# MingSun-Tse/Collaborative-Distillation

Measured on AMD Instinct MI355X. Metric: content megapixels/sec, end-to-end 5-level WCT (16x VGG, 4K content, 2K style), higher is better.
Workload: dtype f32 (f16x3 split-MFMA products, fp32 accumulate); 1 GPU; PytorchWCT/WCT.py --mode 16x, 5-level WCT, 3840x2160 content, 2048x2048 style, alpha=1, style-side work included, images resident in HBM; BASELINE configs[1]; content_total=3840x2160, parallelism=content column strips x1

## Files before the change

collaborative-distillation_amd/csrc/solve.hip:

```cpp
#include "wct_common.h"
#include <cstdlib>

namespace {

typedef double f64x2 __attribute__((ext_vector_type(2)));
typedef unsigned u32x2 __attribute__((ext_vector_type(2)));

constexpr int MAX_SWEEPS = 40;
constexpr double ROT_TOL = 1e-12;
constexpr double ABS_FLOOR = 1e-13;
static const double REL_THRESH = [] { const char* e = wct_debug_env("WCT_REL_THRESH"); return e ? atof(e) : 1e-12; }();

__device__ __forceinline__ void tournament_pair(int n, int round, int k, int& p, int& q) {
  const int m = n - 1;
  if (k == 0) { p = m; q = round % m; }
  else { p = (round + k) % m; q = (round - k + m) % m; }
  if (p > q) { const int t = p; p = q; q = t; }
}

__device__ __forceinline__ double rsqrt_nr(double x) {
  double y = __builtin_amdgcn_rsq(x);
  y = y * (1.5 - 0.5 * x * y * y);
  y = y * (1.5 - 0.5 * x * y * y);
  return y;
// ... 336 lines not shown
    rows[((size_t)o * 9 + t) * cin + c] = v;
    ws += v;
  }
  wsum[e] = ws;
}

constexpr int COOP_NW = 32, COOP_MAXIT = 32;
struct NsSched { double ca[COOP_MAXIT], cb[COOP_MAXIT]; };
struct CoopArgs {
  int C; double n; const double* sum; const double* sumsq; double* res; double diag_add, eps_rel;
  NsWs w; int maxit, inverse; double zmax; int* info; int xcd;
  unsigned* coop_next;
  unsigned* aborts;
};
constexpr int BUF_SC1 = 16;
__device__ __forceinline__ unsigned xcc_id() { unsigned v; asm volatile("s_getreg_b32 %0, hwreg(HW_REG_XCC_ID)" : "=s"(v)); return v & 0xf; }
__device__ __forceinline__ __amdgpu_buffer_rsrc_t coop_rsrc(const void* p) {
  return __builtin_amdgcn_make_buffer_rsrc(const_cast<void*>(p), 0, 128 * 128 * 8, 0x00020000);
}
__device__ __forceinline__ f64x2 coop_ld2(__amdgpu_buffer_rsrc_t r, int elem) {
  return __builtin_bit_cast(f64x2, __builtin_amdgcn_raw_buffer_load_b128(r, elem * 8, 0, BUF_SC1));
}
__device__ __forceinline__ double coop_ld1(__amdgpu_buffer_rsrc_t r, int elem) {
  return __builtin_bit_cast(double, __builtin_amdgcn_raw_buffer_load_b64(r, elem * 8, 0, BUF_SC1));
}
__device__ __forceinline__ void coop_st1(__amdgpu_buffer_rsrc_t r, int elem, double v) {
  __builtin_amdgcn_raw_buffer_store_b64(__builtin_bit_cast(u32x2, v), r, elem * 8, 0, BUF_SC1);
}
__device__ __forceinline__ void gemm32_coop(const double* P, const double* Q, int i0, int j0, int lane, int wave, double (*red)[16 * 64], Acc32& acc) {
  constexpr int CP = 128;
  const int li = lane & 15, kk = lane >> 4, kbeg = wave * (CP / 4);
  const __amdgpu_buffer_rsrc_t rp = coop_rsrc(P), rq = coop_rsrc(Q);
#pragma unroll
  for (int t = 0; t < 4; ++t) acc.t[t] = f64x4{0., 0., 0., 0.};
  const int p0 = (i0 + li) * CP + 4 * kk, p1 = p0 + 16 * CP, q0 = (4 * kk) * CP + j0 + li;
  KBlock x[2];
#pragma unroll
  for (int b = 0; b < 2; ++b) {
    const int k0 = kbeg + 16 * b;
    x[b].a0l = coop_ld2(rp, p0 + k0); x[b].a0h = coop_ld2(rp, p0 + k0 + 2);
    x[b].a1l = coop_ld2(rp, p1 + k0); x[b].a1h = coop_ld2(rp, p1 + k0 + 2);
#pragma unroll
    for (int u = 0; u < 4; ++u) { x[b].b0[u] = coop_ld1(rq, q0 + (k0 + u) * CP); x[b].b1[u] = coop_ld1(rq, q0 + (k0 + u) * CP + 16); }
  }
  kblock_mfma(x[0], acc);
  kblock_mfma(x[1], acc);
  if (wave) {
#pragma unroll
    for (int t = 0; t < 4; ++t)
#pragma unroll
      for (int r = 0; r < 4; ++r) red[wave - 1][(t * 4 + r) * 64 + lane] = acc.t[t][r];
  }
  __syncthreads();
  if (!wave) {
#pragma unroll
    for (int t = 0; t < 4; ++t)
#pragma unroll
      for (int r = 0; r < 4; ++r) {
        const int at = (t * 4 + r) * 64 + lane;
        acc.t[t][r] = ((acc.t[t][r] + red[0][at]) + red[1][at]) + red[2][at];
      }
  }
  __syncthreads();
}
constexpr long long COOP_TIMEOUT_TICKS = 500000ll;
__device__ __forceinline__ void coop_abort(const NsWs& w, unsigned bit, unsigned* aborts) {
  const unsigned old = __hip_atomic_fetch_or(&w.coop[1], bit, __ATOMIC_RELAXED, __HIP_MEMORY_SCOPE_AGENT);
  if (old == 0u && aborts) __hip_atomic_fetch_add(aborts, 1u, __ATOMIC_RELAXED, __HIP_MEMORY_SCOPE_AGENT);
}
__device__ __forceinline__ bool coop_barrier(const NsWs& w, unsigned& target, int* ok_s, unsigned* aborts) {
  __builtin_amdgcn_s_waitcnt(0);
  __syncthreads();
  target += COOP_NW;
  if (threadIdx.x == 0) {
    __hip_atomic_fetch_add(&w.coop[0], 1u, __ATOMIC_RELAXED, __HIP_MEMORY_SCOPE_AGENT);
    const long long t0 = wall_clock64();
    bool ok = true;
    while (__hip_atomic_load(&w.coop[0], __ATOMIC_RELAXED, __HIP_MEMORY_SCOPE_AGENT) < target) {
      if (wall_clock64() - t0 > COOP_TIMEOUT_TICKS || __hip_atomic_load(&w.coop[1], __ATOMIC_RELAXED, __HIP_MEMORY_SCOPE_AGENT)) {
        coop_abort(w, 1u, aborts);
        ok = false;
        break;
      }
      __builtin_amdgcn_s_sleep(1);
    }
    *ok_s = ok;
  }
  __syncthreads();
  return *ok_s != 0;
}

__global__ __launch_bounds__(256) void ns_coop128_kernel(CoopArgs a, NsSched sc) {
  const bool inject = (a.xcd & 16) != 0;
  if ((int)(blockIdx.x & 7) != (a.xcd & 7)) return;
  constexpr int CP = 128;
  __shared__ double red[3][16 * 64];
  __shared__ int sdead[CP];
  __shared__ int ok_s;
  const NsWs& w = a.w;
  const int C = a.C, tid = threadIdx.x, me = blockIdx.x >> 3;
  const int lane = tid & 63, wave = tid >> 6, li = lane & 15, kk = lane >> 4;
  const double n = a.n;
  if (me == 0) {
    if (tid < 4) a.coop_next[tid] = 0u;
// ... 51 lines not shown
    const __amdgpu_buffer_rsrc_t ry = coop_rsrc(w.Y[0]), rz = coop_rsrc(w.Z[0]);
    for (int e = tid; e < 4 * CP; e += 256) {
      const int r = 4 * me + e / CP, c = e % CP;
      double y = r == c ? 1.0 : 0.0;
      if (r < C && c < C) {
        const double cv = cov_value(r, c, C, n, a.sum, a.sumsq, a.diag_add);
        a.res[(size_t)r * C + c] = cv;
        if (c == 0) a.res[(size_t)C * C + C + r] = a.sum[r] / n;
        if (!sdead[r] && !sdead[c]) y = (cv + (r == c ? s1 : 0.0)) / s0;
      }
      coop_st1(ry, r * CP + c, y);
      coop_st1(rz, r * CP + c, r == c ? 1.0 : 0.0);
    }
  }
  unsigned target = 0;
  if (!coop_barrier(w, target, &ok_s, a.aborts)) return;
  if (tid == 0 && (__hip_atomic_load(&w.coop[2], __ATOMIC_RELAXED, __HIP_MEMORY_SCOPE_AGENT) != xcc_id() + 1u || (inject && me == 7)))
    coop_abort(w, 2u, a.aborts);
  if (!coop_barrier(w, target, &ok_s, a.aborts)) return;
  if (__hip_atomic_load(&w.coop[1], __ATOMIC_RELAXED, __HIP_MEMORY_SCOPE_AGENT)) return;
  const int tile = me & 15, zside = me >> 4;
  const int i0 = (tile >> 2) * 32, j0 = (tile & 3) * 32;
  int nit = 0;
  for (int it = 0; it < a.maxit; ++it) {
    if (it > 0 && __longlong_as_double((long long)__hip_atomic_load(&w.resid[it - 1], __ATOMIC_RELAXED, __HIP_MEMORY_SCOPE_AGENT)) < NS_TOL) break;
    const int cur = it & 1, nxt = cur ^ 1;
    if (!zside) {
      Acc32 acc;
      gemm32_coop(w.Z[cur], w.Y[cur], i0, j0, lane, wave, red, acc);
      if (!wave) {
        const __amdgpu_buffer_rsrc_t rt = coop_rsrc(w.T);
        const double ca = sc.ca[it], cb = sc.cb[it];
        double m = 0.;
#pragma unroll
        for (int t = 0; t < 4; ++t)
#pragma unroll
          for (int r = 0; r < 4; ++r) {
            const int row = i0 + 16 * (t >> 1) + kk + 4 * r, col = j0 + 16 * (t & 1) + li;
            const double zy = acc.t[t][r], d = zy - (row == col ? 1.0 : 0.0);
            m = (d == d) ? fmax(m, fabs(d)) : __longlong_as_double(0x7ff0000000000000ll);
            coop_st1(rt, row * CP + col, (row == col ? ca : 0.0) - cb * zy);
          }
        for (int o = 32; o > 0; o >>= 1) m = fmax(m, __shfl_xor(m, o));
        if (lane == 0) atomicMax(&w.resid[it], (unsigned long long)__double_as_longlong(m));
      }
    }
    if (!coop_barrier(w, target, &ok_s, a.aborts)) return;
    {
      Acc32 acc;
      gemm32_coop(zside ? w.T : w.Y[cur], zside ? w.Z[cur] : w.T, i0, j0, lane, wave, red, acc);
      if (!wave) {
        const __amdgpu_buffer_rsrc_t ro = coop_rsrc(zside ? w.Z[nxt] : w.Y[nxt]);
#pragma unroll
        for (int t = 0; t < 4; ++t)
#pragma unroll
          for (int r = 0; r < 4; ++r) coop_st1(ro, (i0 + 16 * (t >> 1) + kk + 4 * r) * CP + j0 + 16 * (t & 1) + li, acc.t[t][r]);
        if (zside) {
          double q = 0.;
#pragma unroll
          for (int t = 0; t < 4; ++t) q += acc.t[t][0] * acc.t[t][0] + acc.t[t][1] * acc.t[t][1] + acc.t[t][2] * acc.t[t][2] + acc.t[t][3] * acc.t[t][3];
          for (int o = 32; o > 0; o >>= 1) q += __shfl_xor(q, o);
          if (lane == 0) atomicAdd(&w.zfro[it + 1], q);
        }
      }
    }
    if (!coop_barrier(w, target, &ok_s, a.aborts)) return;
    nit = it + 1;
  }
  bool ok = nit >= 1 && __longlong_as_double((long long)__hip_atomic_load(&w.resid[nit - 1], __ATOMIC_RELAXED, __HIP_MEMORY_SCOPE_AGENT)) < NS_TOL;
  if (ok && a.inverse) {
    const unsigned long long zb = __hip_atomic_load(reinterpret_cast<unsigned long long*>(&w.zfro[nit]), __ATOMIC_RELAXED, __HIP_MEMORY_SCOPE_AGENT);
    ok = __longlong_as_double((long long)zb) <= a.zmax * a.zmax;
  }
  if (me == 0 && tid == 0) { *w.iters = nit; *w.ok = ok ? 1 : 0; if (a.info && ok) *a.info = nit; }
  if (!ok) return;
  {
    const __amdgpu_buffer_rsrc_t rf = coop_rsrc(a.inverse ? w.Z[nit & 1] : w.Y[nit & 1]);
    const double sc_out = a.inverse ? rsqrt(s0) : sqrt(s0);
    for (int e = tid; e < 4 * CP; e += 256) {
      const int r = 4 * me + e / CP, c = e % CP;
      if (r >= C || c >= C) continue;
      double v = 0.;
      if (!sdead[r] && !sdead[c]) v = coop_ld1(rf, r * CP + c) * sc_out;
// ... 64 lines not shown
  const int li = lane & 15, kk = lane >> 4;
  f64x4 acc = f64x4{0., 0., 0., 0.};
  const double* pp = P + (i0 + li) * LD + kk;
  const double* qq = Q + kk * LD + j0 + li;
#pragma unroll 2
  for (int k0 = 0; k0 < CP; k0 += 16) {
    double a[4], b[4];
#pragma unroll
    for (int u = 0; u < 4; ++u) { a[u] = pp[k0 + 4 * u]; b[u] = qq[(k0 + 4 * u) * LD]; }
#pragma unroll
    for (int u = 0; u < 4; ++u) acc = __builtin_amdgcn_mfma_f64_16x16x4f64(a[u], b[u], acc, 0, 0, 0);
  }
  return acc;
}

template <int CP>
__global__ __launch_bounds__((CP / 16) * (CP / 16) * 64) void ns_lds_kernel(double* res, int C, int inverse, double eps_rel,
                                                                               int maxit, double zmax, int* ok_out, int* info,
                                                                               double npix, const double* sum, const double* sumsq, double diag_add,
                                                                               NsSched sched, int nsched) {
  constexpr int LD = CP + 2, TPR = CP / 16, NW = TPR * TPR, NT = NW * 64;
  extern __shared__ __attribute__((aligned(16))) char smem_ns[];
  double* Y = reinterpret_cast<double*>(smem_ns);
  double* Z = Y + CP * LD;
  double* T = Z + CP * LD;
  double* red = T + CP * LD;
  int* dead = reinterpret_cast<int*>(red + NW + 2);
  const int tid = threadIdx.x, lane = tid & 63, wave = __builtin_amdgcn_readfirstlane(tid >> 6);
  const int li = lane & 15, kk = lane >> 4;
  const int i0 = (wave / TPR) * 16, j0 = (wave % TPR) * 16;
  cov_by_block(C, npix, sum, sumsq, res, diag_add, tid, NT);
// ... 15 lines not shown
  if (!(f > 0.)) f = 1.;
  const double s = f * (1.0 + eps_rel), shift = eps_rel * f;
  for (int e = tid; e < CP * CP; e += NT) {
    const int r = e / CP, c = e - r * CP;
    double y = r == c ? 1.0 : 0.0;
    if (!dead[r] && !dead[c]) y = (res[(size_t)r * C + c] + (r == c ? shift : 0.0)) / s;
    Y[r * LD + c] = y;
    Z[r * LD + c] = r == c ? 1.0 : 0.0;
  }
  __syncthreads();
  int n = 0;
  double prev = 1e300;
  for (int it = 0; it < maxit; ++it) {
    if (it > 0 && prev < NS_TOL) break;
    const double ca = it < nsched ? sched.ca[it] : 1.5, cb = it < nsched ? sched.cb[it] : 0.5;
    const f64x4 zy = tile_gemm_lds<CP>(Z, Y, i0, j0, lane);
    double m = 0.;
#pragma unroll
    for (int r = 0; r < 4; ++r) {
      const int row = i0 + kk + 4 * r, col = j0 + li;
      const double d = zy[r] - (row == col ? 1.0 : 0.0);
      m = (d == d) ? fmax(m, fabs(d)) : __longlong_as_double(0x7ff0000000000000ll);
      T[row * LD + col] = (row == col ? ca : 0.0) - cb * zy[r];
    }
    for (int o = 32; o > 0; o >>= 1) m = fmax(m, __shfl_xor(m, o));
    if (lane == 0) red[wave] = m;
    __syncthreads();
    m = 0.;
    for (int w = 0; w < NW; ++w) m = fmax(m, red[w]);
    prev = m;
    const f64x4 yn = tile_gemm_lds<CP>(Y, T, i0, j0, lane);
    const f64x4 zn = tile_gemm_lds<CP>(T, Z, i0, j0, lane);
    __syncthreads();
#pragma unroll
    for (int r = 0; r < 4; ++r) {
      Y[(i0 + kk + 4 * r) * LD + j0 + li] = yn[r];
      Z[(i0 + kk + 4 * r) * LD + j0 + li] = zn[r];
    }
    __syncthreads();
    n = it + 1;
  }
  bool ok = n >= 1 && prev < NS_TOL;
  if (ok && inverse) {
    double q = 0.;
    for (int e = tid; e < CP * CP; e += NT) { const double z = Z[(e / CP) * LD + (e % CP)]; q += z * z; }
    for (int o = 32; o > 0; o >>= 1) q += __shfl_xor(q, o);
    __syncthreads();
    if (lane == 0) red[wave] = q;
    __syncthreads();
    q = 0.;
    for (int w = 0; w < NW; ++w) q += red[w];
    ok = q <= zmax * zmax;
// ... 224 lines not shown
  for (int j = threadIdx.x; j < n; j += 256) {
    const double l = lam[j];
    wj[j] = (l > thr && l > 0.) ? pow(l, expo - 2.0) : 0.;
  }
  __syncthreads();
  const long e = (long)blockIdx.x * blockDim.x + threadIdx.x;
  if (e >= (long)n * n) return;
  const int a = (int)(e / n), b = (int)(e % n);
  double s = 0.;
  for (int j = 0; j < n; ++j) s += wj[j] * G[(size_t)j * n + a] * G[(size_t)j * n + b];
  out[e] = s;
}

}

size_t eig_result_bytes(int C) { return eig_doubles(C) * sizeof(double); }
size_t eig_result_F_offset(size_t C) { return eig_F_offset((int)C); }
static inline int ns_pad(int C) { return C > 128 ? (C + 63) / 64 * 64 : (C + 31) / 32 * 32; }
size_t eig_workspace_bytes(int C) {
  const size_t cp2 = (size_t)ns_pad(C) * ns_pad(C);
  return 5 * cp2 * sizeof(double) + (size_t)C * sizeof(int) + 4 * sizeof(double) + 2 * (NS_MAXIT_REG + 2) * sizeof(unsigned long long) + 64;
}
size_t assemble_workspace_bytes(int C) { return (size_t)C * C * sizeof(double); }

bool eig_is_big(int C, bool wide_model) { return C > 128 || (wide_model && C > 64 && ns_pad(C) % 64 == 0); }

bool fold_gemm_capable(int cout, int cin, int cout_pad) { return cin >= 256 && cin % 128 == 0 && cout % 32 == 0 && cout_pad == cout; }
size_t fold_gemm_rows_doubles(int cout, int cin) { return (size_t)cout * 10 * cin; }

hipError_t launch_fold_rows(const float* w_oihw, int cout, int cin, double* rows, hipStream_t s) {
// ... 6 lines not shown
                            float* wpk_out, float* bias_out, unsigned* maxbits_dev, hipStream_t s) {
  if (!fold_gemm_capable(cout, cin, cout_pad)) return hipErrorInvalidValue;
  if (maxbits_dev) {
    hipError_t e = hipMemsetAsync(maxbits_dev, 0, sizeof(unsigned), s);
    if (e != hipSuccess) return e;
  }
  constexpr int NS = 8;
  const dim3 grid((unsigned)(cin / 32), (unsigned)(cout * 9 / 32 + (cout_pad + NS - 1) / NS));
  hipLaunchKernelGGL(fold_gemm_kernel<NS>, grid, dim3(64 * NS), 0, s, rows, rows + (size_t)cout * 9 * cin, bias, cout, cin, cout_pad, M, b, wpk_out,
                     bias_out, maxbits_dev);
  return hipGetLastError();
}

hipError_t launch_eig(int C, double n, const double* sum, const double* sumsq, int inverse, double* res, int* info_dev,
                      void* ws, size_t ws_bytes, hipStream_t s, double diag_add, bool wide_model, int* ok_defer, int coop_xcd, unsigned* coop_state, int* coop_epoch,
                      unsigned* coop_aborts, bool* coop_used_out, int sched_maxit, double sched_guess) {
  if (C < 2 || (C & 1) || C > 512 || n < 2) return hipErrorInvalidValue;
  if (ws_bytes < eig_workspace_bytes(C)) return hipErrorOutOfMemory;
  const size_t cc = (size_t)C * C;
  const int Cp = ns_pad(C);
  const size_t cp2 = (size_t)Cp * Cp;
  NsWs w;
  double* p = reinterpret_cast<double*>(ws);
  w.Y[0] = p; w.Y[1] = p + cp2; w.Z[0] = p + 2 * cp2; w.Z[1] = p + 3 * cp2; w.T = p + 4 * cp2;
  w.scal = p + 5 * cp2;
  w.resid = reinterpret_cast<unsigned long long*>(w.scal + 4);
  w.zfro = reinterpret_cast<double*>(w.resid + NS_MAXIT_REG + 2);
  w.iters = reinterpret_cast<int*>(w.zfro + NS_MAXIT_REG + 2);
  w.ok = w.iters + 1;
  w.coop = nullptr;
  w.dead = w.iters + 2;
// ... 15 lines not shown
      hipError_t e = hipFuncSetAttribute(reinterpret_cast<const void*>(kern), hipFuncAttributeMaxDynamicSharedMemorySize, (int)lds);
      if (e != hipSuccess) return e;
      NsSched sc;
      int nsched = 0;
      if (guess64 > 0.) {
        double xl = sqrt(guess64);
        for (; nsched < COOP_MAXIT && nsched < maxit; ++nsched) {
          const double mu = xl <= 0.9 ? sqrt(3.0 / (1.0 + xl + xl * xl)) : 1.0;
          xl = mu * xl * (3.0 - mu * mu * xl * xl) / 2.0;
          sc.ca[nsched] = 1.5 * mu; sc.cb[nsched] = 0.5 * mu * mu * mu;
        }
      }
      hipLaunchKernelGGL(kern, dim3(1), dim3((unsigned)nw * 64), lds, s, res, C, inverse, 1e-15, maxit, NS_ZMAX, w.ok, info_dev, n, sum, sumsq, diag_add, sc, nsched);
      return hipSuccess;
    };
    hipError_t e = Cp == 32 ? go(ns_lds_kernel<32>, 32) : go(ns_lds_kernel<64>, 64);
    if (e != hipSuccess) return e;
  } else {
    static const bool sk_env = [] { const char* e = wct_debug_env("WCT_NS_SPLITK"); return e ? atoi(e) != 0 : true; }();
    const bool splitk128 = sk_env && Cp % 64 == 0;
    const bool coop = !big && Cp == 128 && splitk128 && coop_xcd >= 0 && coop_state && coop_epoch && maxit <= COOP_MAXIT;
    coop_used = coop;
    if (coop_used_out) *coop_used_out = coop;
    if (coop) { w.coop = coop_state + 4 * (*coop_epoch & 1); ++*coop_epoch; }
    if (big) {
      hipLaunchKernelGGL(ns_init_kernel, dim3(1), dim3(1024), 0, s, res, C, NS_DEFLATE, w, maxit);
      hipLaunchKernelGGL(ns_fill_kernel, dim3((unsigned)((cp2 + 255) / 256)), dim3(256), 0, s, res, C, Cp, w);
    } else if (!coop) {
      hipLaunchKernelGGL(ns_prep_kernel, dim3(1), dim3(1024), 0, s, C, Cp, n, sum, sumsq, res, diag_add, 1e-15, w, maxit);
    }
    const dim3 g1(Cp / 32, Cp / 32, 1), g2(Cp / 32, Cp / 32, 2);
// ... 153 lines not shown
```

collaborative-distillation_amd/csrc/wct_api.hip:

```cpp
#include "../../include/wct_hip.h"
#include "../../include/wct_hip_color.h"
#include "../../include/wct_hip_smooth.h"
#include "../../include/wct_hip_swap.h"
#include "../../include/wct_hip_transform.h"
#include "wct_common.h"

#include <cmath>
#include <cstdarg>
#include <cstdlib>
#include <cstdio>
#include <atomic>
#include <cstring>
#include <dlfcn.h>
#include <map>
#include <mutex>
#include <string>
#include <vector>

namespace {

struct DevBuf {
  void* p = nullptr;
  size_t cap = 0;
};
// ... 46 lines not shown
  unsigned coop_solves = 0;
  bool coop_off = false;
};

struct wct_ctx {
  int device = 0;
  Lane main, side;
  hipEvent_t ev_join = nullptr;
  hipEvent_t ev_smom[6] = {nullptr, nullptr, nullptr, nullptr, nullptr, nullptr};
  hipEvent_t ev_sar[6] = {nullptr, nullptr, nullptr, nullptr, nullptr, nullptr};
  hipEvent_t ev_switch = nullptr;
  hipEvent_t ev_fork = nullptr, ev_style[6] = {nullptr, nullptr, nullptr, nullptr, nullptr, nullptr};
  int eig_skip = 0, eig_calls = 0;
  int foldgemm = 1;
  int nscoop = 1;
  int interleave = 1;
  std::string err;
  Module mod[2][6];
  DevBuf featC, featS, tmpT, wsAsm, small, foldW, foldW16, eigC, eigS[6];
  DevBuf foldS[6];
  bool fold_ready[6] = {false, false, false, false, false, false};
  int cur_level = 0, cur_h = 0, cur_w = 0;
  DevBuf u8c, u8s, u8o;
  DevBuf rsz_tmp;
  std::vector<ResizeAxis> rsz_axes;
  unsigned long long rsz_clock = 0;
  DevBuf noise;
  DevBuf colStyle, colOut, colWs;
  DevBuf smSums, smAB;
  DevBuf swFc, swFs, swQ, swK, swOut, swIdx, swRun, swNorm, swLab;
// ... 610 lines not shown
constexpr double OT_GUESS = 1e-10;

int eig_impl(wct_ctx* ctx, Lane& ln, int C, double n, const double* sum, const double* sumsq, int inverse, DevBuf& res, int* info_dev, bool ot_sched = false) {
  if (C < 2 || (C & 1) || C > 512) return fail(ctx, WCT_ERR_INVALID, "solve: C=%d must be even and <= 512", C);
  if (n < 2) return fail(ctx, WCT_ERR_INVALID, "solve: unbiased covariance needs >= 2 pixels (n=%g)", n);
  if (int rc = ensure(ctx, res, eig_result_bytes(C))) return rc;
  if (int rc = ensure(ctx, ln.wsEig, eig_workspace_bytes(C))) return rc;
  if (ctx->eig_skip > 0 && ++ctx->eig_calls > ctx->eig_skip) return WCT_OK;
  ProfScope ps(ctx, ln.stream, inverse ? "matfun_invsqrt" : "matfun_sqrt", 0, 0);
  int* defer = nullptr;
  if (ctx->defer_big && eig_is_big(C, ctx->wide_model) && ctx->ok_n < OK_SLOTS) defer = ctx->ok_log + ctx->ok_n++;
  const bool coop_ok = ctx->nscoop && coop_usable(ctx, ln);
  bool coop_used = false;
  HIPCHK(ctx, launch_eig(C, n, sum, sumsq, inverse, reinterpret_cast<double*>(res.p), info_dev, ln.wsEig.p, ln.wsEig.cap, ln.stream,
                         (inverse && ctx->numpy_variant && !ot_sched) ? 1.0 : 0.0, ctx->wide_model, defer, coop_ok ? (ln.xcd | (ctx->nscoop == 2 ? 16 : 0)) : -1, ln.coop, &ln.coop_epoch,
                         ctx->sat_dev + 2 + (&ln == &ctx->side ? 1 : 0), &coop_used, ot_sched ? OT_MAXIT : 0, ot_sched ? OT_GUESS : -1.0));
  if (coop_used) ++ln.coop_solves;
  return WCT_OK;
}

template <typename BODY>
int with_deferred_solves(wct_ctx* ctx, bool wait_side, BODY&& body) {
  if (!ctx->wide_model) return body();
  ctx->defer_big = true;
  ctx->ok_n = 0;
  HIPCHK(ctx, hipMemcpyAsync(ctx->sat_dev + 1, ctx->sat_dev, sizeof(unsigned), hipMemcpyDeviceToDevice, ctx->main.stream));
  int rc = body();
  ctx->defer_big = false;
  const int n = ctx->ok_n;
  ctx->ok_n = 0;
  if (rc) return rc;
// ... 392 lines not shown

int wct_debug_set(wct_ctx* ctx, const char* key, double value) {
  if (!ctx || !key) return WCT_ERR_INVALID;
  WCT_GUARD(ctx);
  const int v = value != 0.0;
  if (!strcmp(key, "fuse")) ctx->fuse = v;
  else if (!strcmp(key, "sp")) ctx->sp = v;
  else if (!strcmp(key, "l1fuse")) ctx->l1fuse = v;
  else if (!strcmp(key, "u8fuse")) ctx->u8fuse = v;
  else if (!strcmp(key, "upconv")) ctx->upconv = v;
  else if (!strcmp(key, "fastfold")) ctx->fastfold = v;
  else if (!strcmp(key, "interleave")) ctx->interleave = v;
  else if (!strcmp(key, "foldgemm")) ctx->foldgemm = v;
  else if (!strcmp(key, "prof_forms")) ctx->prof_forms = v;
  else if (!strcmp(key, "nscoop")) ctx->nscoop = (int)value;
  else if (!strcmp(key, "mom32")) ctx->mom32 = (int)value;
  else if (!strcmp(key, "in3wide")) ctx->in3wide = (int)value;
  else if (!strcmp(key, "poison")) {
    if (value < 0) { ctx->poison = -1; return WCT_OK; }
    if (value > 255 || value != (double)(int)value) return fail(ctx, WCT_ERR_INVALID, "debug_set: 'poison' takes a byte 0..255, or -1 for off");
    ctx->poison = (int)value;
    return poison_scratch(ctx, ctx->poison);
  }
  else if (!strcmp(key, "eig_skip")) {
    if (!getenv("WCT_DEBUG")) return fail(ctx, WCT_ERR_INVALID, "debug_set: 'eig_skip' produces wrong results by design (timing experiment); set WCT_DEBUG to allow it");
    ctx->eig_skip = (int)value; ctx->eig_calls = 0;
  }
  else if (!strcmp(key, "swap_key_chunk")) {
    if (!getenv("WCT_DEBUG")) return fail(ctx, WCT_ERR_INVALID, "debug_set: 'swap_key_chunk' is a test / measurement key; set WCT_DEBUG to allow it");
    if (value < 0 || value > 2147483647.0 || value != (double)(long)value) return fail(ctx, WCT_ERR_INVALID, "debug_set: 'swap_key_chunk' takes a key count >= 1, or 0 for the default");
// ... 7 lines not shown
    if (!ctx->coll_set || (ctx->comm_ranks != 1 && !ctx->shard_emulate)) return fail(ctx, WCT_ERR_STATE, "debug_set: 'shard_emulate' needs a ONE-rank communicator on the context");
    if (world < 2 || rank >= world) return fail(ctx, WCT_ERR_INVALID, "debug_set: 'shard_emulate' = 100 * ranks + rank");
    ctx->shard_emulate = true; ctx->comm_ranks = world; ctx->comm_rank = rank;
    return WCT_OK;
  }
  else if (!strcmp(key, "side_priority")) {
    int lo = 0, hi = 0;
    HIPCHK(ctx, hipDeviceGetStreamPriorityRange(&lo, &hi));
    HIPCHK(ctx, hipStreamSynchronize(ctx->side.stream));
    hipStream_t ns = nullptr;
    HIPCHK(ctx, hipStreamCreateWithPriority(&ns, hipStreamNonBlocking, value > 0 ? lo : (value < 0 ? hi : 0)));
    (void)hipStreamDestroy(ctx->side.stream);
    ctx->side.stream = ns;
    return WCT_OK;
  }
  else return fail(ctx, WCT_ERR_INVALID, "debug_set: unknown key '%s' (fuse, sp, l1fuse, u8fuse, upconv, fastfold, interleave, foldgemm, nscoop, in3wide, mom32, eig_skip, side_priority, poison, prof_forms, swap_key_chunk)", key);
  HIPCHK(ctx, hipStreamSynchronize(ctx->side.stream));
  return WCT_OK;
}

int wct_debug_get(wct_ctx* ctx, const char* key, double* value) {
  if (!ctx || !key || !value) return WCT_ERR_INVALID;
  WCT_GUARD(ctx);
  if (!strcmp(key, "nscoop_aborts") || !strcmp(key, "nscoop_solves") || !strcmp(key, "nscoop_off")) {
    if (!strcmp(key, "nscoop_solves")) { *value = (double)ctx->main.coop_solves + (double)ctx->side.coop_solves; return WCT_OK; }
    if (!strcmp(key, "nscoop_off")) { (void)coop_usable(ctx, ctx->main); (void)coop_usable(ctx, ctx->side); *value = (ctx->main.coop_off ? 1 : 0) + (ctx->side.coop_off ? 2 : 0); return WCT_OK; }
    HIPCHK(ctx, hipStreamSynchronize(ctx->side.stream));
    HIPCHK(ctx, hipStreamSynchronize(ctx->main.stream));
    unsigned n[2] = {0u, 0u};
    HIPCHK(ctx, hipMemcpy(n, ctx->sat_dev + 2, sizeof n, hipMemcpyDeviceToHost));
    if (ctx->sat_host) { reinterpret_cast<volatile unsigned*>(ctx->sat_host)[2] = n[0]; reinterpret_cast<volatile unsigned*>(ctx->sat_host)[3] = n[1]; }
// ... 1800 lines not shown
```

collaborative-distillation_amd/csrc/wct_common.h:

```cpp
#pragma once
#include <hip/hip_runtime.h>
#include <stdint.h>
#include <stddef.h>

#include <stdlib.h>
#include <vector>

typedef float f32x4 __attribute__((ext_vector_type(4)));
typedef double f64x4 __attribute__((ext_vector_type(4)));

static inline const char* wct_debug_env(const char* name) {
  const char* g = getenv("WCT_DEBUG");
  if (!g || !g[0] || (g[0] == '0' && !g[1])) return nullptr;
  return getenv(name);
}

struct LaunchForm { char form; int tile_h; bool multi; };
extern __thread LaunchForm wct_launch_form __attribute__((visibility("hidden")));
static inline void note_launch_form(char form, int tile_h, long units, long grid) {
  wct_launch_form.form = form; wct_launch_form.tile_h = tile_h; wct_launch_form.multi = units > grid;
}

__device__ __forceinline__ void sat_raise(unsigned* counter) {
  const unsigned old = atomicAdd(counter, 1u);
// ... 104 lines not shown
hipError_t launch_nhwc_to_nchw(const float* in, float* out, int C, int npix, hipStream_t s);
hipError_t launch_nchw_to_nhwc(const float* in, float* out, int C, int npix, hipStream_t s);

size_t moments_workspace_bytes(int C, long npix);
hipError_t launch_moments(const float* feat_nhwc, int C, int h, int wfull, int x0, int x1, double* sum,
                          double* sumsq, void* workspace, size_t workspace_bytes, hipStream_t s, bool f32_products = false);

size_t eig_result_bytes(int C);
size_t eig_result_F_offset(size_t C);
size_t eig_workspace_bytes(int C);
size_t assemble_workspace_bytes(int C);
bool eig_is_big(int C, bool wide_model);
hipError_t launch_eig(int C, double n, const double* sum, const double* sumsq, int inverse, double* res, int* info_dev,
                      void* workspace, size_t workspace_bytes, hipStream_t s, double diag_add = 0.0, bool wide_model = false,
                      int* ok_defer = nullptr, int coop_xcd = -1, unsigned* coop_state = nullptr, int* coop_epoch = nullptr, unsigned* coop_aborts = nullptr, bool* coop_used_out = nullptr,
                      int sched_maxit = 0, double sched_guess = -1.0);
hipError_t launch_assemble(int C, const double* eig_c, const double* eig_s, double alpha, double rel_thresh,
                           double* M, double* b, void* workspace, size_t workspace_bytes, hipStream_t s);

size_t ot_workspace_bytes(int C);
hipError_t launch_ot_sandwich(int C, double n, const double* sum_c, const double* sumsq_c, const double* S, double* B, double* zeros, double* tmp, hipStream_t s);
hipError_t launch_ot_assemble(int C, double alpha, const double* S, const double* mu_s, const double* Z, double n, const double* sum_c, double* tmp,
                              double* M, double* b, hipStream_t s);
hipError_t launch_adain_assemble(int C, double alpha, double eps, const double* S, const double* mu_s, double n, const double* sum_c, const double* sumsq_c,
                                 double* M, double* b, int* info_dev, hipStream_t s);

bool fold_gemm_capable(int cout, int cin, int cout_pad);
size_t fold_gemm_rows_doubles(int cout, int cin);
hipError_t launch_fold_rows(const float* w_oihw, int cout, int cin, double* rows, hipStream_t s);
hipError_t launch_fold_gemm(const double* rows, const float* bias, int cout, int cin, int cout_pad, const double* M, const double* b,
                            float* wpk_out, float* bias_out, unsigned* maxbits_dev, hipStream_t s);
// ... 34 lines not shown
```

Before: 1158 MP/s.

## Overlap Newton-Schulz operand loads with grid barriers and split LDS solver work

The cooperative Newton-Schulz kernel's grid barrier is split into arrive and wait, so operand loads for the second GEMM that do not depend on T are issued before the wait. The barrier poll reads the counter and abort flag together in one 64-bit load, one redundant barrier is removed, and the residual is cached per iteration. The single-block LDS solver gains a new form, on by default, that splits waves between the Y and Z updates and prefetches operands before the sync. Both kernels now use a DPP-based wave max reduction. Optional timing instrumentation is added under a compile flag.

Measured after the change: 1144 MP/s. -1.2%, worse.

```diff
diff --git a/collaborative-distillation_amd/csrc/solve.hip b/collaborative-distillation_amd/csrc/solve.hip
--- a/collaborative-distillation_amd/csrc/solve.hip
+++ b/collaborative-distillation_amd/csrc/solve.hip
@@ -5,6 +5,23 @@
 
 typedef double f64x2 __attribute__((ext_vector_type(2)));
 typedef unsigned u32x2 __attribute__((ext_vector_type(2)));
+
+template <int CTRL>
+__device__ __forceinline__ double dpp_f64(double v) {
+  const int lo = __builtin_amdgcn_update_dpp(0, __double2loint(v), CTRL, 0xf, 0xf, false);
+  const int hi = __builtin_amdgcn_update_dpp(0, __double2hiint(v), CTRL, 0xf, 0xf, false);
+  return __hiloint2double(hi, lo);
+}
+__device__ __forceinline__ double wave_fmax(double m) {
+  m = fmax(m, dpp_f64<0xB1>(m));
+  m = fmax(m, dpp_f64<0x4E>(m));
+  m = fmax(m, dpp_f64<0x141>(m));
+  m = fmax(m, dpp_f64<0x140>(m));
+  double r[4];
+#pragma unroll
+  for (int q = 0; q < 4; ++q) r[q] = __hiloint2double(__builtin_amdgcn_readlane(__double2hiint(m), 16 * q), __builtin_amdgcn_readlane(__double2loint(m), 16 * q));
+  return fmax(fmax(r[0], r[1]), fmax(r[2], r[3]));
+}
 
 constexpr int MAX_SWEEPS = 40;
 constexpr double ROT_TOL = 1e-12;
@@ -374,6 +391,26 @@
   unsigned* aborts;
 };
 constexpr int BUF_SC1 = 16;
+enum { NS_T_LOAD1, NS_T_MMA1, NS_T_RED1, NS_T_STORE1, NS_T_BAR1, NS_T_LOAD2, NS_T_MMA2, NS_T_RED2, NS_T_STORE2, NS_T_BAR2, NS_T_FRONT, NS_T_BAR0, NS_T_ITERS, NS_T_SLOTS };
+#ifdef WCT_NS_TIMING
+__device__ unsigned long long g_ns_t[2][NS_T_SLOTS];
+struct NsClk {
+  unsigned long long t[NS_T_SLOTS]; long long last; bool on;
+  __device__ void start(bool who) { on = who && threadIdx.x == 0; for (int i = 0; i < NS_T_SLOTS; ++i) t[i] = 0; last = wall_clock64(); }
+  __device__ __forceinline__ void stamp(int i) {
+    if (on) { __builtin_amdgcn_sched_barrier(0); const long long c = wall_clock64(); t[i] += (unsigned long long)(c - last); last = c; __builtin_amdgcn_sched_barrier(0); }
+  }
+  __device__ __forceinline__ void landed() { __builtin_amdgcn_s_waitcnt(0); }
+  __device__ void flush(int bank) { if (on) for (int i = 0; i < NS_T_SLOTS; ++i) atomicAdd(&g_ns_t[bank][i], t[i]); }
+};
+#else
+struct NsClk {
+  __device__ __forceinline__ void start(bool) {}
+  __device__ __forceinline__ void stamp(int) {}
+  __device__ __forceinline__ void landed() {}
+  __device__ __forceinline__ void flush(int) {}
+};
+#endif
 __device__ __forceinline__ unsigned xcc_id() { unsigned v; asm volatile("s_getreg_b32 %0, hwreg(HW_REG_XCC_ID)" : "=s"(v)); return v & 0xf; }
 __device__ __forceinline__ __amdgpu_buffer_rsrc_t coop_rsrc(const void* p) {
   return __builtin_amdgcn_make_buffer_rsrc(const_cast<void*>(p), 0, 128 * 128 * 8, 0x00020000);
@@ -387,24 +424,38 @@
 __device__ __forceinline__ void coop_st1(__amdgpu_buffer_rsrc_t r, int elem, double v) {
   __builtin_amdgcn_raw_buffer_store_b64(__builtin_bit_cast(u32x2, v), r, elem * 8, 0, BUF_SC1);
 }
-__device__ __forceinline__ void gemm32_coop(const double* P, const double* Q, int i0, int j0, int lane, int wave, double (*red)[16 * 64], Acc32& acc) {
+__device__ __forceinline__ void coop_load_a(KBlock (&x)[2], const double* P, int i0, int lane, int wave) {
   constexpr int CP = 128;
   const int li = lane & 15, kk = lane >> 4, kbeg = wave * (CP / 4);
-  const __amdgpu_buffer_rsrc_t rp = coop_rsrc(P), rq = coop_rsrc(Q);
-#pragma unroll
-  for (int t = 0; t < 4; ++t) acc.t[t] = f64x4{0., 0., 0., 0.};
-  const int p0 = (i0 + li) * CP + 4 * kk, p1 = p0 + 16 * CP, q0 = (4 * kk) * CP + j0 + li;
-  KBlock x[2];
+  const __amdgpu_buffer_rsrc_t rp = coop_rsrc(P);
+  const int p0 = (i0 + li) * CP + 4 * kk, p1 = p0 + 16 * CP;
 #pragma unroll
   for (int b = 0; b < 2; ++b) {
     const int k0 = kbeg + 16 * b;
     x[b].a0l = coop_ld2(rp, p0 + k0); x[b].a0h = coop_ld2(rp, p0 + k0 + 2);
     x[b].a1l = coop_ld2(rp, p1 + k0); x[b].a1h = coop_ld2(rp, p1 + k0 + 2);
+  }
+}
+__device__ __forceinline__ void coop_load_b(KBlock (&x)[2], const double* Q, int j0, int lane, int wave) {
+  constexpr int CP = 128;
+  const int li = lane & 15, kk = lane >> 4, kbeg = wave * (CP / 4);
+  const __amdgpu_buffer_rsrc_t rq = coop_rsrc(Q);
+  const int q0 = (4 * kk) * CP + j0 + li;
+#pragma unroll
+  for (int b = 0; b < 2; ++b) {
+    const int k0 = kbeg + 16 * b;
 #pragma unroll
     for (int u = 0; u < 4; ++u) { x[b].b0[u] = coop_ld1(rq, q0 + (k0 + u) * CP); x[b].b1[u] = coop_ld1(rq, q0 + (k0 + u) * CP + 16); }
   }
+}
+__device__ __forceinline__ void coop_mma(const KBlock (&x)[2], int lane, int wave, double (*red)[16 * 64], Acc32& acc, NsClk& clk, int slot) {
+  clk.landed();
+  clk.stamp(slot);
+#pragma unroll
+  for (int t = 0; t < 4; ++t) acc.t[t] = f64x4{0., 0., 0., 0.};
   kblock_mfma(x[0], acc);
   kblock_mfma(x[1], acc);
+  clk.stamp(slot + 1);
   if (wave) {
 #pragma unroll
     for (int t = 0; t < 4; ++t)
@@ -422,32 +473,44 @@
       }
   }
   __syncthreads();
+  clk.stamp(slot + 2);
 }
 constexpr long long COOP_TIMEOUT_TICKS = 500000ll;
 __device__ __forceinline__ void coop_abort(const NsWs& w, unsigned bit, unsigned* aborts) {
   const unsigned old = __hip_atomic_fetch_or(&w.coop[1], bit, __ATOMIC_RELAXED, __HIP_MEMORY_SCOPE_AGENT);
   if (old == 0u && aborts) __hip_atomic_fetch_add(aborts, 1u, __ATOMIC_RELAXED, __HIP_MEMORY_SCOPE_AGENT);
 }
-__device__ __forceinline__ bool coop_barrier(const NsWs& w, unsigned& target, int* ok_s, unsigned* aborts) {
+__device__ __forceinline__ void coop_arrive(const NsWs& w, unsigned& target, NsClk& clk, int slot) {
   __builtin_amdgcn_s_waitcnt(0);
+  clk.stamp(slot - 1);
   __syncthreads();
   target += COOP_NW;
+  if (threadIdx.x == 0) __hip_atomic_fetch_add(&w.coop[0], 1u, __ATOMIC_RELAXED, __HIP_MEMORY_SCOPE_AGENT);
+}
+__device__ __forceinline__ bool coop_wait(const NsWs& w, unsigned target, int* ok_s, unsigned* aborts, NsClk& clk, int slot) {
   if (threadIdx.x == 0) {
-    __hip_atomic_fetch_add(&w.coop[0], 1u, __ATOMIC_RELAXED, __HIP_MEMORY_SCOPE_AGENT);
     const long long t0 = wall_clock64();
     bool ok = true;
-    while (__hip_atomic_load(&w.coop[0], __ATOMIC_RELAXED, __HIP_MEMORY_SCOPE_AGENT) < target) {
-      if (wall_clock64() - t0 > COOP_TIMEOUT_TICKS || __hip_atomic_load(&w.coop[1], __ATOMIC_RELAXED, __HIP_MEMORY_SCOPE_AGENT)) {
+    for (;;) {
+      const unsigned long long st = __hip_atomic_load(reinterpret_cast<unsigned long long*>(w.coop), __ATOMIC_RELAXED, __HIP_MEMORY_SCOPE_AGENT);
+      const bool here = (unsigned)st >= target;
+      if ((unsigned)(st >> 32) || (!here && wall_clock64() - t0 > COOP_TIMEOUT_TICKS)) {
         coop_abort(w, 1u, aborts);
         ok = false;
         break;
       }
+      if (here) break;
       __builtin_amdgcn_s_sleep(1);
     }
     *ok_s = ok;
   }
   __syncthreads();
+  clk.stamp(slot);
   return *ok_s != 0;
+}
+__device__ __forceinline__ bool coop_barrier(const NsWs& w, unsigned& target, int* ok_s, unsigned* aborts, NsClk& clk, int slot) {
+  coop_arrive(w, target, clk, slot);
+  return coop_wait(w, target, ok_s, aborts, clk, slot);
 }
 
 __global__ __launch_bounds__(256) void ns_coop128_kernel(CoopArgs a, NsSched sc) {
@@ -529,20 +592,25 @@
     }
   }
   unsigned target = 0;
-  if (!coop_barrier(w, target, &ok_s, a.aborts)) return;
+  NsClk clk;
+  clk.start(me == 0 || me == 16);
+  if (!coop_barrier(w, target, &ok_s, a.aborts, clk, NS_T_BAR0)) return;
   if (tid == 0 && (__hip_atomic_load(&w.coop[2], __ATOMIC_RELAXED, __HIP_MEMORY_SCOPE_AGENT) != xcc_id() + 1u || (inject && me == 7)))
     coop_abort(w, 2u, a.aborts);
-  if (!coop_barrier(w, target, &ok_s, a.aborts)) return;
-  if (__hip_atomic_load(&w.coop[1], __ATOMIC_RELAXED, __HIP_MEMORY_SCOPE_AGENT)) return;
   const int tile = me & 15, zside = me >> 4;
   const int i0 = (tile >> 2) * 32, j0 = (tile & 3) * 32;
   int nit = 0;
+  unsigned long long rprev = 0ull;
   for (int it = 0; it < a.maxit; ++it) {
-    if (it > 0 && __longlong_as_double((long long)__hip_atomic_load(&w.resid[it - 1], __ATOMIC_RELAXED, __HIP_MEMORY_SCOPE_AGENT)) < NS_TOL) break;
+    if (it > 0 && __longlong_as_double((long long)rprev) < NS_TOL) break;
     const int cur = it & 1, nxt = cur ^ 1;
+    KBlock x2[2];
     if (!zside) {
       Acc32 acc;
-      gemm32_coop(w.Z[cur], w.Y[cur], i0, j0, lane, wave, red, acc);
+      KBlock x1[2];
+      coop_load_a(x1, w.Z[cur], i0, lane, wave);
+      coop_load_b(x1, w.Y[cur], j0, lane, wave);
+      coop_mma(x1, lane, wave, red, acc, clk, NS_T_LOAD1);
       if (!wave) {
         const __amdgpu_buffer_rsrc_t rt = coop_rsrc(w.T);
         const double ca = sc.ca[it], cb = sc.cb[it];
@@ -556,14 +624,20 @@
             m = (d == d) ? fmax(m, fabs(d)) : __longlong_as_double(0x7ff0000000000000ll);
             coop_st1(rt, row * CP + col, (row == col ? ca : 0.0) - cb * zy);
           }
-        for (int o = 32; o > 0; o >>= 1) m = fmax(m, __shfl_xor(m, o));
+        m = wave_fmax(m);
         if (lane == 0) atomicMax(&w.resid[it], (unsigned long long)__double_as_longlong(m));
       }
     }
-    if (!coop_barrier(w, target, &ok_s, a.aborts)) return;
+    coop_arrive(w, target, clk, NS_T_BAR1);
+    if (zside) coop_load_b(x2, w.Z[cur], j0, lane, wave);
+    else coop_load_a(x2, w.Y[cur], i0, lane, wave);
+    if (!coop_wait(w, target, &ok_s, a.aborts, clk, NS_T_BAR1)) return;
+    rprev = __hip_atomic_load(&w.resid[it], __ATOMIC_RELAXED, __HIP_MEMORY_SCOPE_AGENT);
     {
       Acc32 acc;
-      gemm32_coop(zside ? w.T : w.Y[cur], zside ? w.Z[cur] : w.T, i0, j0, lane, wave, red, acc);
+      if (zside) coop_load_a(x2, w.T, i0, lane, wave);
+      else coop_load_b(x2, w.T, j0, lane, wave);
+      coop_mma(x2, lane, wave, red, acc, clk, NS_T_LOAD2);
       if (!wave) {
         const __amdgpu_buffer_rsrc_t ro = coop_rsrc(zside ? w.Z[nxt] : w.Y[nxt]);
 #pragma unroll
@@ -579,9 +653,13 @@
         }
       }
     }
-    if (!coop_barrier(w, target, &ok_s, a.aborts)) return;
+    if (!coop_barrier(w, target, &ok_s, a.aborts, clk, NS_T_BAR2)) return;
     nit = it + 1;
   }
+#ifdef WCT_NS_TIMING
+  if (clk.on) clk.t[NS_T_ITERS] = (unsigned long long)nit;
+  clk.flush(me == 0 ? 0 : 1);
+#endif
   bool ok = nit >= 1 && __longlong_as_double((long long)__hip_atomic_load(&w.resid[nit - 1], __ATOMIC_RELAXED, __HIP_MEMORY_SCOPE_AGENT)) < NS_TOL;
   if (ok && a.inverse) {
     const unsigned long long zb = __hip_atomic_load(reinterpret_cast<unsigned long long*>(&w.zfro[nit]), __ATOMIC_RELAXED, __HIP_MEMORY_SCOPE_AGENT);
@@ -676,7 +754,38 @@
   return acc;
 }
 
+template <int CP, int Q0 = 0, int Q1 = CP / 4>
+__device__ __forceinline__ void lds_load_a(double (&a)[CP / 4], const double* P, int i0, int lane) {
+  const double* pp = P + (i0 + (lane & 15)) * (CP + 2) + (lane >> 4);
+#pragma unroll
+  for (int q = Q0; q < Q1; ++q) a[q] = pp[4 * q];
+}
+template <int CP, int Q0 = 0, int Q1 = CP / 4>
+__device__ __forceinline__ void lds_load_b(double (&b)[CP / 4], const double* Q, int j0, int lane) {
+  const double* qq = Q + (lane >> 4) * (CP + 2) + j0 + (lane & 15);
+#pragma unroll
+  for (int q = Q0; q < Q1; ++q) b[q] = qq[4 * q * (CP + 2)];
+}
 template <int CP>
+__device__ __forceinline__ f64x4 lds_mma(const double (&a)[CP / 4], const double (&b)[CP / 4]) {
+  f64x4 acc = f64x4{0., 0., 0., 0.};
+#pragma unroll
+  for (int q = 0; q < CP / 4; ++q) acc = __builtin_amdgcn_mfma_f64_16x16x4f64(a[q], b[q], acc, 0, 0, 0);
+  return acc;
+}
+template <int CP>
+__device__ __forceinline__ void lds_mma2(const double (&a0)[CP / 4], const double (&b0)[CP / 4], const double (&a1)[CP / 4], const double (&b1)[CP / 4],
+                                         f64x4& acc0, f64x4& acc1) {
+  acc0 = f64x4{0., 0., 0., 0.};
+  acc1 = f64x4{0., 0., 0., 0.};
+#pragma unroll
+  for (int q = 0; q < CP / 4; ++q) {
+    acc0 = __builtin_amdgcn_mfma_f64_16x16x4f64(a0[q], b0[q], acc0, 0, 0, 0);
+    acc1 = __builtin_amdgcn_mfma_f64_16x16x4f64(a1[q], b1[q], acc1, 0, 0, 0);
+  }
+}
+
+template <int CP, int FORM>
 __global__ __launch_bounds__((CP / 16) * (CP / 16) * 64) void ns_lds_kernel(double* res, int C, int inverse, double eps_rel,
                                                                                int maxit, double zmax, int* ok_out, int* info,
                                                                                double npix, const double* sum, const double* sumsq, double diag_add,
@@ -722,7 +831,14 @@
   for (int it = 0; it < maxit; ++it) {
     if (it > 0 && prev < NS_TOL) break;
     const double ca = it < nsched ? sched.ca[it] : 1.5, cb = it < nsched ? sched.cb[it] : 0.5;
-    const f64x4 zy = tile_gemm_lds<CP>(Z, Y, i0, j0, lane);
+    f64x4 zy;
+    if constexpr (FORM == 0) zy = tile_gemm_lds<CP>(Z, Y, i0, j0, lane);
+    else {
+      double za[CP / 4], yb[CP / 4];
+      lds_load_a<CP>(za, Z, i0, lane);
+      lds_load_b<CP>(yb, Y, j0, lane);
+      zy = lds_mma<CP>(za, yb);
+    }
     double m = 0.;
 #pragma unroll
     for (int r = 0; r < 4; ++r) {
@@ -731,19 +847,53 @@
       m = (d == d) ? fmax(m, fabs(d)) : __longlong_as_double(0x7ff0000000000000ll);
       T[row * LD + col] = (row == col ? ca : 0.0) - cb * zy[r];
     }
-    for (int o = 32; o > 0; o >>= 1) m = fmax(m, __shfl_xor(m, o));
+    if constexpr (FORM == 0) { for (int o = 32; o > 0; o >>= 1) m = fmax(m, __shfl_xor(m, o)); }
+    else m = wave_fmax(m);
     if (lane == 0) red[wave] = m;
-    __syncthreads();
-    m = 0.;
-    for (int w = 0; w < NW; ++w) m = fmax(m, red[w]);
-    prev = m;
-    const f64x4 yn = tile_gemm_lds<CP>(Y, T, i0, j0, lane);
-    const f64x4 zn = tile_gemm_lds<CP>(T, Z, i0, j0, lane);
-    __syncthreads();
-#pragma unroll
-    for (int r = 0; r < 4; ++r) {
-      Y[(i0 + kk + 4 * r) * LD + j0 + li] = yn[r];
-      Z[(i0 + kk + 4 * r) * LD + j0 + li] = zn[r];
+    if constexpr (FORM == 0) {
+      __syncthreads();
+      m = 0.;
+      for (int w = 0; w < NW; ++w) m = fmax(m, red[w]);
+      prev = m;
+      const f64x4 yn = tile_gemm_lds<CP>(Y, T, i0, j0, lane);
+      const f64x4 zn = tile_gemm_lds<CP>(T, Z, i0, j0, lane);
+      __syncthreads();
+#pragma unroll
+      for (int r = 0; r < 4; ++r) {
+        Y[(i0 + kk + 4 * r) * LD + j0 + li] = yn[r];
+        Z[(i0 + kk + 4 * r) * LD + j0 + li] = zn[r];
+      }
+    } else {
+      constexpr int HALF = NW / 2;
+      const bool zs = wave >= HALF;
+      const int p = zs ? wave - HALF : wave;
+      const int ia = zs ? (p / (TPR / 2)) * 16 : (p / TPR) * 32, jb = zs ? (p % (TPR / 2)) * 32 : (p % TPR) * 16;
+      double o0[CP / 4], o1[CP / 4], tt[CP / 4];
+      constexpr int NQ = CP / 4, PF = CP == 64 ? NQ / 4 : NQ;
+      if (zs) { lds_load_b<CP, 0, PF>(o0, Z, jb, lane); lds_load_b<CP, 0, PF>(o1, Z, jb + 16, lane); }
+      else { lds_load_a<CP, 0, PF>(o0, Y, ia, lane); lds_load_a<CP, 0, PF>(o1, Y, ia + 16, lane); }
+      __syncthreads();
+      m = 0.;
+      for (int w = 0; w < NW; ++w) m = fmax(m, red[w]);
+      prev = m;
+      f64x4 n0, n1;
+      if (zs) {
+        lds_load_a<CP>(tt, T, ia, lane);
+        lds_load_b<CP, PF, NQ>(o0, Z, jb, lane); lds_load_b<CP, PF, NQ>(o1, Z, jb + 16, lane);
+        lds_mma2<CP>(tt, o0, tt, o1, n0, n1);
+      } else {
+        lds_load_b<CP>(tt, T, jb, lane);
+        lds_load_a<CP, PF, NQ>(o0, Y, ia, lane); lds_load_a<CP, PF, NQ>(o1, Y, ia + 16, lane);
+        lds_mma2<CP>(o0, tt, o1, tt, n0, n1);
+      }
+      __syncthreads();
+      double* out = zs ? Z : Y;
+      const int ib = zs ? ia : ia + 16, jc = zs ? jb + 16 : jb;
+#pragma unroll
+      for (int r = 0; r < 4; ++r) {
+        out[(ia + kk + 4 * r) * LD + jb + li] = n0[r];
+        out[(ib + kk + 4 * r) * LD + jc + li] = n1[r];
+      }
     }
     __syncthreads();
     n = it + 1;
@@ -998,6 +1148,14 @@
 
 }
 
+#ifdef WCT_NS_TIMING
+extern "C" int wct_debug_ns_timing(unsigned long long* out) {
+  unsigned long long z[2][NS_T_SLOTS] = {};
+  if (hipMemcpyFromSymbol(out, HIP_SYMBOL(g_ns_t), sizeof(z)) != hipSuccess) return -1;
+  return hipMemcpyToSymbol(HIP_SYMBOL(g_ns_t), z, sizeof(z)) == hipSuccess ? NS_T_SLOTS : -1;
+}
+#endif
+
 size_t eig_result_bytes(int C) { return eig_doubles(C) * sizeof(double); }
 size_t eig_result_F_offset(size_t C) { return eig_F_offset((int)C); }
 static inline int ns_pad(int C) { return C > 128 ? (C + 63) / 64 * 64 : (C + 31) / 32 * 32; }
@@ -1034,7 +1192,7 @@
 
 hipError_t launch_eig(int C, double n, const double* sum, const double* sumsq, int inverse, double* res, int* info_dev,
                       void* ws, size_t ws_bytes, hipStream_t s, double diag_add, bool wide_model, int* ok_defer, int coop_xcd, unsigned* coop_state, int* coop_epoch,
-                      unsigned* coop_aborts, bool* coop_used_out, int sched_maxit, double sched_guess) {
+                      unsigned* coop_aborts, bool* coop_used_out, int sched_maxit, double sched_guess, int lds_form) {
   if (C < 2 || (C & 1) || C > 512 || n < 2) return hipErrorInvalidValue;
   if (ws_bytes < eig_workspace_bytes(C)) return hipErrorOutOfMemory;
   const size_t cc = (size_t)C * C;
@@ -1080,7 +1238,8 @@
       hipLaunchKernelGGL(kern, dim3(1), dim3((unsigned)nw * 64), lds, s, res, C, inverse, 1e-15, maxit, NS_ZMAX, w.ok, info_dev, n, sum, sumsq, diag_add, sc, nsched);
       return hipSuccess;
     };
-    hipError_t e = Cp == 32 ? go(ns_lds_kernel<32>, 32) : go(ns_lds_kernel<64>, 64);
+    hipError_t e = lds_form ? (Cp == 32 ? go(ns_lds_kernel<32, 1>, 32) : go(ns_lds_kernel<64, 1>, 64))
+                            : (Cp == 32 ? go(ns_lds_kernel<32, 0>, 32) : go(ns_lds_kernel<64, 0>, 64));
     if (e != hipSuccess) return e;
   } else {
     static const bool sk_env = [] { const char* e = wct_debug_env("WCT_NS_SPLITK"); return e ? atoi(e) != 0 : true; }();
diff --git a/collaborative-distillation_amd/csrc/wct_api.hip b/collaborative-distillation_amd/csrc/wct_api.hip
--- a/collaborative-distillation_amd/csrc/wct_api.hip
+++ b/collaborative-distillation_amd/csrc/wct_api.hip
@@ -84,6 +84,7 @@
   int eig_skip = 0, eig_calls = 0;
   int foldgemm = 1;
   int nscoop = 1;
+  int nslds = 1;
   int interleave = 1;
   std::string err;
   Module mod[2][6];
@@ -724,7 +725,7 @@
   bool coop_used = false;
   HIPCHK(ctx, launch_eig(C, n, sum, sumsq, inverse, reinterpret_cast<double*>(res.p), info_dev, ln.wsEig.p, ln.wsEig.cap, ln.stream,
                          (inverse && ctx->numpy_variant && !ot_sched) ? 1.0 : 0.0, ctx->wide_model, defer, coop_ok ? (ln.xcd | (ctx->nscoop == 2 ? 16 : 0)) : -1, ln.coop, &ln.coop_epoch,
-                         ctx->sat_dev + 2 + (&ln == &ctx->side ? 1 : 0), &coop_used, ot_sched ? OT_MAXIT : 0, ot_sched ? OT_GUESS : -1.0));
+                         ctx->sat_dev + 2 + (&ln == &ctx->side ? 1 : 0), &coop_used, ot_sched ? OT_MAXIT : 0, ot_sched ? OT_GUESS : -1.0, ctx->nslds));
   if (coop_used) ++ln.coop_solves;
   return WCT_OK;
 }
@@ -1147,6 +1148,7 @@
   else if (!strcmp(key, "foldgemm")) ctx->foldgemm = v;
   else if (!strcmp(key, "prof_forms")) ctx->prof_forms = v;
   else if (!strcmp(key, "nscoop")) ctx->nscoop = (int)value;
+  else if (!strcmp(key, "nslds")) ctx->nslds = v;
   else if (!strcmp(key, "mom32")) ctx->mom32 = (int)value;
   else if (!strcmp(key, "in3wide")) ctx->in3wide = (int)value;
   else if (!strcmp(key, "poison")) {
@@ -1184,7 +1186,7 @@
     ctx->side.stream = ns;
     return WCT_OK;
   }
-  else return fail(ctx, WCT_ERR_INVALID, "debug_set: unknown key '%s' (fuse, sp, l1fuse, u8fuse, upconv, fastfold, interleave, foldgemm, nscoop, in3wide, mom32, eig_skip, side_priority, poison, prof_forms, swap_key_chunk)", key);
+  else return fail(ctx, WCT_ERR_INVALID, "debug_set: unknown key '%s' (fuse, sp, l1fuse, u8fuse, upconv, fastfold, interleave, foldgemm, nscoop, nslds, in3wide, mom32, eig_skip, side_priority, poison, prof_forms, swap_key_chunk)", key);
   HIPCHK(ctx, hipStreamSynchronize(ctx->side.stream));
   return WCT_OK;
 }
diff --git a/collaborative-distillation_amd/csrc/wct_common.h b/collaborative-distillation_amd/csrc/wct_common.h
--- a/collaborative-distillation_amd/csrc/wct_common.h
+++ b/collaborative-distillation_amd/csrc/wct_common.h
@@ -142,7 +142,7 @@
 hipError_t launch_eig(int C, double n, const double* sum, const double* sumsq, int inverse, double* res, int* info_dev,
                       void* workspace, size_t workspace_bytes, hipStream_t s, double diag_add = 0.0, bool wide_model = false,
                       int* ok_defer = nullptr, int coop_xcd = -1, unsigned* coop_state = nullptr, int* coop_epoch = nullptr, unsigned* coop_aborts = nullptr, bool* coop_used_out = nullptr,
-                      int sched_maxit = 0, double sched_guess = -1.0);
+                      int sched_maxit = 0, double sched_guess = -1.0, int lds_form = 1);
 hipError_t launch_assemble(int C, const double* eig_c, const double* eig_s, double alpha, double rel_thresh,
                            double* M, double* b, void* workspace, size_t workspace_bytes, hipStream_t s);
 
diff --git a/collaborative-distillation_amd/k.s b/collaborative-distillation_amd/k.s
--- /dev/null
+++ b/collaborative-distillation_amd/k.s
@@ -0,0 +1 @@
+
```
